# MDProject/Binary-Fluctuating-Lattice-Boltzmann

Hardware: AMD Instinct MI355X
Metric: MLUPS (million lattice-site updates/sec) D3Q19×2 at 256³/512³; % HBM roofline (higher is better)
Workload: dtype f64; 1 GPU; 512x512x512 periodic, stripe init, zero noise; schedule=handover, slab_per_gpu=512x512x512, parallelism=single GPU

## Files before the change

binary-fluctuating-lattice-boltzmann_amd/_lib.py:

```python
import ctypes
import os

_HERE = os.path.dirname(os.path.abspath(__file__))
LIB_PATH = os.environ.get("BFLBM_LIB", os.path.join(_HERE, "csrc", "libbflbm.so"))

NVEL = 19
NHYDRO = 22
NHYDROBAR = 9
TRACE_NREC = 12
HALO_STATE, HALO_NEXT, HALO_UPLOAD = 0, 1, 2


class Params(ctypes.Structure):
    _fields_ = [
        ("tau_f", ctypes.c_double), ("tau_g", ctypes.c_double),
        ("alpha0", ctypes.c_double), ("alpha1", ctypes.c_double),
        ("kappa", ctypes.c_double), ("kBT", ctypes.c_double), ("cs2", ctypes.c_double),
        ("rho_lo", ctypes.c_double), ("rho_hi", ctypes.c_double),
        ("seed", ctypes.c_uint64),
    ]


class Domain(ctypes.Structure):
    _fields_ = [
# ... 40 lines not shown
    "bflbm_ring_set_overlap": (ctypes.c_int, [_vp, ctypes.c_int]),
    "bflbm_ring_set_transport": (ctypes.c_int, [_vp, ctypes.c_int]),
    "bflbm_ring_last_transport": (ctypes.c_int, [_vp, _P(ctypes.c_int), _P(ctypes.c_int)]),
    "bflbm_debug_addresses": (ctypes.c_int, [_vp, _P(ctypes.c_ulonglong)]),
    "bflbm_tune_placement": (ctypes.c_int, [_vp, ctypes.c_int, _P(ctypes.c_float), _P(ctypes.c_int)]),
    "bflbm_placement_report": (ctypes.c_int, [_vp, _P(ctypes.c_float), _P(ctypes.c_int), _P(ctypes.c_int)]),
    "bflbm_state_total_max": (ctypes.c_int, [_vp, _dp]),
    "bflbm_set_state_total_max": (ctypes.c_int, [_vp, ctypes.c_double]),
    "bflbm_step_boundary": (ctypes.c_int, [_vp]),
    "bflbm_step_interior": (ctypes.c_int, [_vp]),
    "bflbm_step_finish": (ctypes.c_int, [_vp]),
    "bflbm_halo_bytes": (ctypes.c_int, [_vp, ctypes.c_int, _P(ctypes.c_size_t)]),
    "bflbm_halo_pack": (ctypes.c_int, [_vp, ctypes.c_int, ctypes.c_int, _vp]),
    "bflbm_halo_unpack": (ctypes.c_int, [_vp, ctypes.c_int, ctypes.c_int, _vp]),
    "bflbm_halo_planes": (ctypes.c_int, [_vp, ctypes.c_int, ctypes.c_int, ctypes.c_int, _P(_vp), _P(ctypes.c_size_t), _P(ctypes.c_int)]),
    "bflbm_ring_create": (ctypes.c_int, [_P(Params), _P(ctypes.c_int), ctypes.c_int, _P(ctypes.c_int), ctypes.c_int, _P(_vp)]),
    "bflbm_ring_destroy": (ctypes.c_int, [_vp]),
    "bflbm_ring_size": (ctypes.c_int, [_vp, _P(ctypes.c_int)]),
    "bflbm_ring_slab": (ctypes.c_int, [_vp, ctypes.c_int, _P(_vp)]),
    "bflbm_ring_set_params": (ctypes.c_int, [_vp, _P(Params)]),
    "bflbm_ring_set_schedule": (ctypes.c_int, [_vp, ctypes.c_int]),
    "bflbm_ring_init_mixture": (ctypes.c_int, [_vp]),
    "bflbm_ring_init_stripe": (ctypes.c_int, [_vp, ctypes.c_double]),
    "bflbm_ring_init_droplet": (ctypes.c_int, [_vp, ctypes.c_double]),
    "bflbm_ring_commit_upload": (ctypes.c_int, [_vp, ctypes.c_int]),
    "bflbm_ring_step": (ctypes.c_int, [_vp, ctypes.c_int]),
    "bflbm_ring_com_sums": (ctypes.c_int, [_vp, _dp]),
    "bflbm_ring_mass": (ctypes.c_int, [_vp, _dp, _dp]),
    "bflbm_ring_sync": (ctypes.c_int, [_vp]),
    "bflbm_ring_set_ref_state": (ctypes.c_int, [_vp, _vp, _vp, _vp, _P(Fab)]),
    "bflbm_ring_enable_ref_state": (ctypes.c_int, [_vp, ctypes.c_int, _dp]),
    "bflbm_ring_prepare_ref": (ctypes.c_int, [_vp]),
    "bflbm_batch_create": (ctypes.c_int, [_P(Params), ctypes.c_int, _P(ctypes.c_int), ctypes.c_int, _P(_vp)]),
    "bflbm_batch_destroy": (ctypes.c_int, [_vp]),
    "bflbm_batch_size": (ctypes.c_int, [_vp, _P(ctypes.c_int)]),
    "bflbm_batch_replica": (ctypes.c_int, [_vp, ctypes.c_int, _P(_vp)]),
    "bflbm_batch_set_schedule": (ctypes.c_int, [_vp, ctypes.c_int]),
    "bflbm_batch_resolved_schedule": (ctypes.c_int, [_vp, _P(ctypes.c_int)]),
    "bflbm_batch_step": (ctypes.c_int, [_vp, ctypes.c_int]),
    "bflbm_batch_sync": (ctypes.c_int, [_vp]),
    "bflbm_trace_create": (ctypes.c_int, [_vp, ctypes.c_int, ctypes.c_longlong, ctypes.c_double, _P(_vp)]),
    "bflbm_batch_trace_create": (ctypes.c_int, [_vp, ctypes.c_int, ctypes.c_longlong, ctypes.c_double, _P(_vp)]),
    "bflbm_trace_destroy": (ctypes.c_int, [_vp]),
    "bflbm_trace_sample": (ctypes.c_int, [_vp]),
    "bflbm_trace_reset": (ctypes.c_int, [_vp]),
    "bflbm_trace_count": (ctypes.c_int, [_vp, _P(ctypes.c_longlong), _P(ctypes.c_int)]),
    "bflbm_trace_read": (ctypes.c_int, [_vp, ctypes.c_longlong, ctypes.c_longlong, _vp, _vp]),
    "bflbm_set_ref_state": (ctypes.c_int, [_vp, _vp, _vp, _vp, _P(Fab)]),
    "bflbm_enable_ref_state": (ctypes.c_int, [_vp, ctypes.c_int, _dp]),
    "bflbm_ref_state_active": (ctypes.c_int, [_vp, _P(ctypes.c_int)]),
    "bflbm_set_com": (ctypes.c_int, [_vp, _dp]),
    "bflbm_get_hydrovsbar": (ctypes.c_int, [_vp, _vp, ctypes.c_int, _P(Fab)]),
    "bflbm_get_hydrovs": (ctypes.c_int, [_vp, _vp, ctypes.c_int, _P(Fab)]),
    "bflbm_get_noise": (ctypes.c_int, [_vp, _vp, _vp, _P(Fab)]),
    "bflbm_inject_noise": (ctypes.c_int, [_vp, _vp, _vp, _P(Fab)]),
    "bflbm_com_sums": (ctypes.c_int, [_vp, _dp]),
    "bflbm_mass": (ctypes.c_int, [_vp, _dp, _dp]),
    "bflbm_sync": (ctypes.c_int, [_vp]),
    "bflbm_droplet_moments": (ctypes.c_int, [_vp, _dp]),
    "bflbm_ring_droplet_moments": (ctypes.c_int, [_vp, _dp]),
    "bflbm_fit_droplet": (ctypes.c_int, [_vp, _dp, _dp, ctypes.c_int, ctypes.c_double, _dp, _P(ctypes.c_int)]),
    "bflbm_ring_fit_droplet": (ctypes.c_int, [_vp, _dp, _dp, ctypes.c_int, ctypes.c_double, _dp, _P(ctypes.c_int)]),
    "bflbm_flowfit_default_opts": (None, [_P(FlowFitOpts)]),
    "bflbm_fit_droplet_flow": (ctypes.c_int, [_vp, _P(FlowFitOpts), _dp, _P(ctypes.c_int)]),
    "bflbm_ring_fit_droplet_flow": (ctypes.c_int, [_vp, _P(FlowFitOpts), _dp, _P(ctypes.c_int)]),
    "bflbm_flowfit_coefficients": (ctypes.c_int, [ctypes.c_double] * 6 + [_dp]),
    "bflbm_sf_create": (ctypes.c_int, [_vp, ctypes.c_int, _P(ctypes.c_int), _P(ctypes.c_int), _dp, _P(_vp)]),
    "bflbm_sf_destroy": (ctypes.c_int, [_vp]),
    "bflbm_sf_reset": (ctypes.c_int, [_vp]),
    "bflbm_sf_accumulate": (ctypes.c_int, [_vp, ctypes.c_int, ctypes.c_int]),
    "bflbm_sf_nsamples": (ctypes.c_int, [_vp, _P(ctypes.c_longlong)]),
    "bflbm_sf_get": (ctypes.c_int, [_vp, ctypes.c_int, ctypes.c_int, _vp]),
    "bflbm_ring_sf_create": (ctypes.c_int, [_vp, ctypes.c_int, _P(ctypes.c_int), _P(ctypes.c_int), _dp, _P(_vp)]),
    "bflbm_ring_sf_destroy": (ctypes.c_int, [_vp]),
    "bflbm_ring_sf_reset": (ctypes.c_int, [_vp]),
    "bflbm_ring_sf_accumulate": (ctypes.c_int, [_vp, ctypes.c_int, ctypes.c_int]),
    "bflbm_ring_sf_nsamples": (ctypes.c_int, [_vp, _P(ctypes.c_longlong)]),
    "bflbm_ring_sf_get": (ctypes.c_int, [_vp, ctypes.c_int, ctypes.c_int, _vp]),
    "bflbm_timer_start": (ctypes.c_int, [_vp]),
    "bflbm_timer_stop": (ctypes.c_int, [_vp, _P(ctypes.c_float)]),
    "bflbm_rng_site_normals": (ctypes.c_int, [ctypes.c_uint64, ctypes.c_uint64, ctypes.c_uint32, _dp]),
    "bflbm_debug_time_kernel": (ctypes.c_int, [_vp, ctypes.c_int, ctypes.c_int, _P(ctypes.c_float)]),
    "bflbm_device_bytes": (ctypes.c_int, [_vp, _P(ctypes.c_size_t)]),
}


class BflbmError(RuntimeError):
    pass


_lib = None


def load():
    global _lib
    if _lib is not None:
        return _lib
    if not os.path.exists(LIB_PATH):
        raise BflbmError(
            f"{LIB_PATH} not found: build the HIP extension first "
            "(python -c 'import __graft_entry__ as g; g.build()' or make -C "
            f"{os.path.dirname(LIB_PATH)}). There is no CPU fallback.")
    if os.environ.get("BFLBM_NO_TORCH") != "1":
        try:
            import torch
        except ImportError:
            pass
    lib = ctypes.CDLL(LIB_PATH)
    for name, (res, args) in SIGNATURES.items():
        fn = getattr(lib, name)
        fn.restype = res
        fn.argtypes = args
    if lib.bflbm_abi_version() != 1:
        raise BflbmError("libbflbm.so ABI version mismatch")
    _lib = lib
    return lib


def check(rc):
    if rc != 0:
        msg = load().bflbm_last_error()
        raise BflbmError(msg.decode() if msg else f"bflbm call failed ({rc})")
```

binary-fluctuating-lattice-boltzmann_amd/csrc/bflbm.hip:

```cpp
#include <hip/hip_runtime.h>
#include <algorithm>
#include <array>
#include <cmath>
#include <cstdarg>
#include <cstdio>
#include <cstring>
#include <limits>
#include <string>
#include <thread>
#include <vector>

#include "../../include/bflbm.h"
#define BFLBM_NHYDRO_ 22
#include "bflbm_kernels.h"
#include "bflbm_fused.h"
#include "bflbm_handover.h"
#include "bflbm_batch.h"

namespace {

thread_local std::string g_err;

int fail(const char* fmt, ...) {
  char buf[512];
// ... 955 lines not shown
  return 0;
}

int bflbm_ref_state_active(const bflbm_ctx* c, int* active) {
  if (!c || !active) return fail("null argument");
  *active = ref_active(c) ? 1 : 0;
  return 0;
}

int bflbm_set_com(bflbm_ctx* c, const double com[3]) {
  if (!c || !com) return fail("null argument");
  BFLBM_REFUSE_OPEN_STEP(c, "bflbm_set_com");
  for (int d = 0; d < 3; ++d) if (!std::isfinite(com[d])) return fail("bflbm_set_com: centre of mass is not finite");
  for (int d = 0; d < 3; ++d) c->com[d] = com[d];
  c->com_valid = true;
  return 0;
}

int bflbm_sync(bflbm_ctx* c) {
  if (!c) return fail("null context");
  HIP_TRY(hipSetDevice(c->dom.device));
  HIP_TRY(hipStreamSynchronize(c->stream));
  return 0;
}

int bflbm_timer_start(bflbm_ctx* c) {
  if (!c) return fail("null context");
  HIP_TRY(hipEventRecord(c->ev0, c->stream));
  return 0;
}
int bflbm_timer_stop(bflbm_ctx* c, float* ms) {
  if (!c || !ms) return fail("null argument");
  HIP_TRY(hipEventRecord(c->ev1, c->stream));
  HIP_TRY(hipEventSynchronize(c->ev1));
  HIP_TRY(hipEventElapsedTime(ms, c->ev0, c->ev1));
  return 0;
}

int bflbm_rng_site_normals(uint64_t seed, uint64_t site, uint32_t noise_index, double* out36) {
  if (!out36) return fail("null argument");
  static const double tab[BFLBM_NORMAL_TABLE_N] = BFLBM_NORMAL_TABLE_VALUES;
  bflbm_rng_state st;
  bflbm_rng_seed((uint32_t)seed, (uint32_t)(seed >> 32), site, noise_index, st);
  for (int k = 0; k < 36; ++k) out36[k] = (k < 33) ? bflbm_normal_from_bits(bflbm_rng_next(st), tab) : 0.;
  return 0;
}

int bflbm_debug_time_kernel(bflbm_ctx* c, int which, int reps, float* ms) {
  if (!c || !ms || reps < 1) return fail("bad argument");
  if (c->step_open()) return fail("diagnostics inside an open step");
  HIP_TRY(hipSetDevice(c->dom.device));
  const size_t sbytes = (size_t)2 * Q * c->G.vol * sizeof(double);
  for (int r = -1; r < reps; ++r) {
    if (r == 0) HIP_TRY(hipEventRecord(c->ev0, c->stream));
    if (which == 0) hipLaunchKernelGGL(k_pull, plane_grid(c, c->nzl), dim3(256), 0, c->stream, c->S[c->cur], c->S[1 - c->cur], c->G, own_lo(c));
    else if (which == 1) hipLaunchKernelGGL(k_density, plane_grid(c, c->nzl), dim3(256), 0, c->stream, c->S[c->cur], c->rho, c->phi, c->G, own_lo(c));
    else if (which == 2) HIP_TRY(hipMemcpyAsync(c->S[1 - c->cur], c->S[c->cur], sbytes, hipMemcpyDeviceToDevice, c->stream));
    else return fail("unknown diagnostic kernel %d", which);
  }
  HIP_TRY(hipGetLastError());
  HIP_TRY(hipEventRecord(c->ev1, c->stream));
  HIP_TRY(hipEventSynchronize(c->ev1));
  float t = 0.f;
  HIP_TRY(hipEventElapsedTime(&t, c->ev0, c->ev1));
  *ms = t / reps;
  halos_written(c);
  return 0;
}


int bflbm_debug_addresses(const bflbm_ctx* c, unsigned long long out[8]) {
  if (!c || !out) return fail("null argument");
  out[0] = (unsigned long long)c->S[0]; out[1] = (unsigned long long)c->S[1]; out[2] = (unsigned long long)c->rho; out[3] = (unsigned long long)c->phi;
  out[4] = (unsigned long long)c->partial; out[5] = (unsigned long long)c->frames[0]; out[6] = (unsigned long long)c->frames[1]; out[7] = (unsigned long long)c->G.vol;
  return 0;
}

int bflbm_device_bytes(const bflbm_ctx* c, size_t* bytes) {
  if (!c || !bytes) return fail("null argument");
  *bytes = c->bytes;
  return 0;
}


struct bflbm_ring {
  std::vector<bflbm_ctx*> ctx;
  std::vector<hipStream_t> comm;
  std::vector<hipEvent_t> packed;
  std::vector<hipEvent_t> unpacked;
  std::vector<std::array<bool, 2>> peer_ok;
  size_t bytes = 0;
  bool overlap = true;
  int transport = 0;
  int last_kernel_faces = 0, last_copy_faces = 0;
};

static int ring_mark(bflbm_ring* r) {
  const int n = (int)r->ctx.size();
  if (n == 1) return 0;
  for (int k = 0; k < n; ++k) {
    bflbm_ctx* c = r->ctx[k];
    HIP_TRY(hipSetDevice(c->dom.device));
    HIP_TRY(hipEventRecord(r->packed[k], c->stream));
  }
  return 0;
}
static int ring_copy(bflbm_ring* r, int kind) {
  const int n = (int)r->ctx.size();
  if (n == 1) return 0;
  r->last_kernel_faces = r->last_copy_faces = 0;
  for (int k = 0; k < n; ++k) {
    bflbm_ctx* c = r->ctx[k];
    const int lower = (k + n - 1) % n, upper = (k + 1) % n;
    HIP_TRY(hipSetDevice(c->dom.device));
    HIP_TRY(hipStreamWaitEvent(r->comm[k], r->packed[lower], 0));
    HIP_TRY(hipStreamWaitEvent(r->comm[k], r->packed[upper], 0));
    HIP_TRY(hipStreamWaitEvent(r->comm[k], r->packed[k], 0));
    const size_t pbytes = (size_t)c->G.plane * sizeof(double);
    for (int side = 0; side < 2; ++side) {
      bflbm_ctx* src = r->ctx[side == 0 ? lower : upper];
      HaloTable Tu, Tp;
      halo_table(c, kind, side, false, Tu);
      halo_table(src, kind, 1 - side, true, Tp);
      double* dst_base = halo_buffer(c, kind);
      const double* src_base = halo_buffer(src, kind);
      for (int e = 0; e < 2 * Q; ++e) if (Tu.comp[e] != Tp.comp[e]) return fail("halo tables of neighbouring slabs disagree");
      static const bool force_copies = [] { const char* e = getenv("BFLBM_RING_COPY_FALLBACK"); return e && atoi(e) != 0; }();
      const bool reachable = !force_copies && r->transport == 0 && ((src->dom.device == c->dom.device) || r->peer_ok[k][side]);
      if (reachable && (c->G.plane % 2 == 0) && (c->G.vol % 2 == 0) && (src->G.vol % 2 == 0)) {
        ++r->last_kernel_faces;
        dim3 g((unsigned)((c->G.plane / 2 + 255) / 256), (unsigned)(2 * Q));
        hipLaunchKernelGGL(k_halo_pull, g, dim3(256), 0, r->comm[k], dst_base, src_base, c->G.plane, c->G.vol, src->G.vol, Tu, Tp);
        HIP_TRY(hipGetLastError());
      } else {
        ++r->last_copy_faces;
        for (int e = 0; e < 2 * Q; ++e) {
          double* d = dst_base + (size_t)Tu.comp[e] * c->G.vol + (size_t)Tu.plane[e] * c->G.plane;
          const double* sp = src_base + (size_t)Tp.comp[e] * src->G.vol + (size_t)Tp.plane[e] * src->G.plane;
          HIP_TRY(hipMemcpyPeerAsync(d, c->dom.device, sp, src->dom.device, pbytes, r->comm[k]));
        }
      }
    }
    HIP_TRY(hipEventRecord(r->unpacked[k], r->comm[k]));
    if (kind == BFLBM_HALO_STATE) halos_written(c);
  }
  return 0;
}
static int ring_exchange(bflbm_ring* r, int kind) { return ring_mark(r) || ring_copy(r, kind); }

static int ring_join(bflbm_ring* r) {
  const int n = (int)r->ctx.size();
  if (n == 1) return 0;
  for (int k = 0; k < n; ++k) {
    HIP_TRY(hipSetDevice(r->ctx[k]->dom.device));
    HIP_TRY(hipStreamWaitEvent(r->ctx[k]->stream, r->unpacked[k], 0));
    HIP_TRY(hipStreamWaitEvent(r->ctx[k]->stream, r->unpacked[(k + 1) % n], 0));
    HIP_TRY(hipStreamWaitEvent(r->ctx[k]->stream, r->unpacked[(k + n - 1) % n], 0));
  }
  return 0;
}

int bflbm_ring_create(const bflbm_params* p, const int n[3], int nslabs, const int* devices, int ndevices, bflbm_ring** out) {
  if (!p || !n || !out || nslabs < 1) return fail("bflbm_ring_create: bad argument");
  if (nslabs > 1 && n[2] / nslabs < 4) return fail("bflbm_ring_create: every slab needs at least 4 planes");
  bflbm_ring* r = new bflbm_ring();
  for (int k = 0; k < nslabs; ++k) {
// ... 365 lines not shown
```

binary-fluctuating-lattice-boltzmann_amd/csrc/bflbm_handover_body.inc:

```
  using L = HoLayout<TY>;
  constexpr int TX = 64, NT = TX * TY;
  constexpr int LW = TX + 2, LSZ = (TX + 2) * (TY + 2);
  constexpr int NRING = 2 * (TX + 2) + 2 * TY;
  static_assert(TY >= 4 && 4 + 2 * TY <= 64 && 8 * TY <= 64, "tile shape");
  __shared__ double rp[4][2][LSZ];
  __shared__ double gl[Q][NT];
  __shared__ double fl[Q][NT];
  __shared__ double exch[2][2][2][2][TX];
  __shared__ double accs[2][2][2][TX];
  __shared__ double colacc[2][2][2][TY][6];
  __shared__ double colfin[2][2][2][TY][6];

  __shared__ double ntab[MODE == 1 ? BFLBM_NORMAL_TABLE_N : 4];

  int col, chunk;
  if (!fused_map(F, (int)blockIdx.x, col, chunk)) return;
  if (MODE == 1) d_load_normal_table(ntab, true);
  const int tix = col % F.ntx;
  int tiy = col / F.ntx + F.row0;
  if (tiy >= F.nty) tiy -= F.nty;
  const int x0 = tix * TX, y0 = tiy * TY;
  const int tid = threadIdx.x;
  const int lane = tid & 63;
  const int ty = __builtin_amdgcn_readfirstlane(tid >> 6);
// ... 48 lines not shown
    }
  }

  const int qa = F.pa + chunk * F.cstride;
  const int qb = min(F.pb, qa + F.lz);
  auto wrapp = [&](int q) {
    if (!G.zwrap) return q;
    const int m = q % G.nzs;
    return m < 0 ? m + G.nzs : m;
  };
  const int fa = qa + 1, fb = qb - 2;

  double anb[2][2] = {{0., 0.}, {0., 0.}};
  double aup[2][2] = {{0., 0.}, {0., 0.}};

  auto finish = [&](int tpf, int rb) {
    if (tpf < fa || tpf > fb) return;
    double* __restrict__ fp = Hg.fout + (long long)tpf * Hg.fplane;
    if (!RAG) {
      if (edge_row) {
#pragma unroll
        for (int k = 0; k < 2; ++k) {
          const double e = exch[rb][k][side_y][0][lane] + exch[rb][k][side_y][1][lane];
          st(fp, tile_rec + (unsigned)(k * L::FR + (side_y ? L::ET : L::EB) + lane) * 8u, e);
        }
      }
    } else {
#pragma unroll
      for (int k = 0; k < 2; ++k) {
        if (r_bot) st(fp, tile_rec + (unsigned)(k * L::FR + L::EB + lane) * 8u, exch[rb][k][0][0][lane] + exch[rb][k][0][1][lane]);
        if (r_top) st(fp, tile_rec + (unsigned)(k * L::FR + L::ET + lane) * 8u, exch[rb][k][1][0][lane] + exch[rb][k][1][1][lane]);
      }
    }
    if (ty == 0 && lane < 8 * TY) {
      const int k = lane / (4 * TY), rem = lane % (4 * TY), sd = rem / (2 * TY), u = rem % (2 * TY);
      const int ne = ah > 2 ? ah - 2 : 0;
      double v = 0.; int slot = -1;
      if (u < ne) {
        const int row = u + 1;
        v = colfin[rb][k][sd][row][0] + colfin[rb][k][sd][row - 1][1] + colfin[rb][k][sd][row + 1][2];
        slot = (sd ? L::ER : L::EL) + row - 1;
      } else if (u - ne < ah + 2) {
        const int row = u - ne - 1;
        if (row >= 0 && row < ah) v = colfin[rb][k][sd][row][3];
        if (row - 1 >= 0 && row - 1 < ah) v += colfin[rb][k][sd][row - 1][4];
        if (row + 1 >= 0 && row + 1 < ah) v += colfin[rb][k][sd][row + 1][5];
        slot = (sd ? L::OR_ : L::OL) + row + 1;
      }
      if (slot >= 0) st(fp, tile_rec + (unsigned)(k * L::FR + slot) * 8u, v);
    }
  };

  auto pull_plane = [&](int q, double (&f)[Q], double (&g)[Q], double (&hv)[2][4], const int which = 0, const int parts = 3) {
    const double* __restrict__ pl[3] = { S + (long long)wrapp(q - 1) * G.plane, S + (long long)wrapp(q) * G.plane,
                                         S + (long long)wrapp(q + 1) * G.plane };
    unsigned oo[3][3];
#pragma unroll
    for (int a = 0; a < 3; ++a)
#pragma unroll
      for (int b2 = 0; b2 < 3; ++b2) { oo[a][b2] = yo[a] + xo[b2]; asm volatile("" : "+v"(oo[a][b2])); }
    if (parts & 1) {
#pragma unroll
      for (int i = 0; i < Q; ++i) {
        const double* __restrict__ b = pl[1 - Vel::cz[i]] + (long long)i * G.vol;
        const unsigned o = oo[1 - Vel::cy[i]][1 - Vel::cx[i]];
        if (which != 2) f[i] = ld(b, o);
        if (which != 1) g[i] = ld(b + (long long)Q * G.vol, o);
      }
    }
    if ((parts & 2) && which != 2 && Hg.use_frames && q >= fa && q <= fb && has_rtask) {
      const double* __restrict__ fp = Hg.fin + (long long)q * Hg.fplane;
#pragma unroll
      for (int j = 0; j < 4; ++j) {
        unsigned o = fo[j];
        asm volatile("" : "+v"(o));
        if (j < 2 || j < nfo) { hv[0][j] = ld(fp, o); hv[1][j] = ld(fp + L::FR, o); }
        else { hv[0][j] = 0.; hv[1][j] = 0.; }
      }
    }
  };
  double nf[Q], ng[Q], hvn[2][4];
  constexpr bool DEFER_G = UNIT && MODE == 0 && !RAG;
  double dg[Q];
  pull_plane(qa - 1, nf, ng, hvn);
  __builtin_amdgcn_s_waitcnt(0x0F70);

  int it = 0;
  auto position = [&](const int q, auto col_c, auto ldn_c, auto pend_c, auto keep_c) {
    constexpr bool do_collide = decltype(col_c)::value, load_next = decltype(ldn_c)::value;
    constexpr bool pending = decltype(pend_c)::value, keep = decltype(keep_c)::value;
    constexpr bool spread_f = do_collide && load_next;
    const int slot = it & 3;
    const double* __restrict__ pl[3] = { S + (long long)wrapp(q - 1) * G.plane, S + (long long)wrapp(q) * G.plane,
                                         S + (long long)wrapp(q + 1) * G.plane };
    double cf[Q], cg[Q], hv[2][4];
#pragma unroll
    for (int i = 0; i < Q; ++i) { cf[i] = nf[i]; cg[i] = ng[i]; }
#pragma unroll
    for (int j = 0; j < 4; ++j) { hv[0][j] = hvn[0][j]; hv[1][j] = hvn[1][j]; }
    const bool ring_from_frames = Hg.use_frames && q >= fa && q <= fb;
    double zero = 0.0;
    asm volatile("" : "+v"(zero));
    auto density = [&](const double (&fs)[Q]) { double r = zero;
#pragma unroll
      for (int i = 0; i < Q; ++i) r += fs[i];
      return r; };
    if (ring_from_frames) {
      if (active) { rp[slot][0][lown] = density(cf); rp[slot][1][lown] = density(cg); }
      if (has_rtask) {
        double r0 = hv[0][0] + hv[0][1], r1 = hv[1][0] + hv[1][1];
        if (nfo > 2) { r0 += hv[0][2]; r1 += hv[1][2]; }
        if (nfo > 3) { r0 += hv[0][3]; r1 += hv[1][3]; }
        rp[slot][0][lhalo] = r0; rp[slot][1][lhalo] = r1;
      }
    } else {
      if (active) { rp[slot][0][lown] = density(cf); rp[slot][1][lown] = density(cg); }
      if (tid < (RAG ? 2 * (aw + 2) + 2 * ah : NRING)) {
        const int r = tid;
        int rx, ry;
        if (r < aw + 2) { rx = r; ry = 0; }
        else if (r < 2 * (aw + 2)) { rx = r - (aw + 2); ry = ah + 1; }
        else if (r < 2 * (aw + 2) + ah) { rx = 0; ry = r - 2 * (aw + 2) + 1; }
        else { rx = aw + 1; ry = r - 2 * (aw + 2) - ah + 1; }
        const int hx = wrapx(x0 + rx - 1), hy = wrapy(y0 + ry - 1);
        const unsigned hxo[3] = { (unsigned)wrapx(hx - 1) * 8u, (unsigned)hx * 8u, (unsigned)wrapx(hx + 1) * 8u };
        const unsigned hyo[3] = { (unsigned)(wrapy(hy - 1) * G.pitch) * 8u, (unsigned)(hy * G.pitch) * 8u, (unsigned)(wrapy(hy + 1) * G.pitch) * 8u };
        double t[2][Q];
#pragma unroll
        for (int i = 0; i < Q; ++i) {
          unsigned o = hyo[1 - Vel::cy[i]] + hxo[1 - Vel::cx[i]];
          asm volatile("" : "+v"(o));
          const double* __restrict__ b = pl[1 - Vel::cz[i]] + (long long)i * G.vol;
          t[0][i] = ld(b, o);
          t[1][i] = ld(b + (long long)Q * G.vol, o);
        }
        __builtin_amdgcn_sched_barrier(0);
        rp[slot][0][ry * LW + rx] = density(t[0]);
        rp[slot][1][ry * LW + rx] = density(t[1]);
      }
    }
    if (pending) {
      double* __restrict__ Dq = D + (long long)wrapp(q - 2) * G.plane + (long long)Q * G.vol;
      unsigned oq = yo[1] + xo[1];
#pragma unroll
      for (int i = 0; i < Q; ++i) {
        if (!ho_g_deferred(i)) continue;
        asm volatile("" : "+v"(oq));
        __builtin_nontemporal_store(dg[i], reinterpret_cast<double*>(reinterpret_cast<char*>(Dq + (long long)i * G.vol) + oq));
      }
    }
    __syncthreads();
    finish(q - 3, (it & 1) ^ 1);
    const int pc = q - 1;
    double mg[Q], jg[3];
    if (do_collide) {
      double pg[Q];
#pragma unroll
      for (int i = 0; i < Q; ++i) pg[i] = gl[i][tid];
      d_moments(pg, mg);
      d_momentum(pg, jg);
    }
    double mf[Q], jf[3];
    if (do_collide) {
      double pfl[Q];
#pragma unroll
      for (int i = 0; i < Q; ++i) pfl[i] = fl[i][tid];
      d_moments(pfl, mf);
      d_momentum(pfl, jf);
    }
#pragma unroll
    for (int i = 0; i < Q; ++i) gl[i][tid] = cg[i];
#pragma unroll
    for (int i = 0; i < Q; ++i) fl[i][tid] = cf[i];
    if (load_next) pull_plane(q + 1, nf, ng, hvn, 1, spread_f ? 2 : 3);
    if (do_collide) {
      const int sl[3] = { (it - 2) & 3, (it - 1) & 3, it & 3 };
      const double r = rp[sl[1]][0][lown], ph = rp[sl[1]][1][lown];
      double nb[Q], grad_rho[3], grad_phi[3];
#pragma unroll
      for (int i = 0; i < Q; ++i) nb[i] = rp[sl[1 + Vel::cz[i]]][0][lown + Vel::cy[i] * LW + Vel::cx[i]];
      d_gradient(P, nb, grad_rho);
#pragma unroll
      for (int i = 0; i < Q; ++i) nb[i] = rp[sl[1 + Vel::cz[i]]][1][lown + Vel::cy[i] * LW + Vel::cx[i]];
      d_gradient(P, nb, grad_phi);
      const int pcw = wrapp(pc);
      double fn3[3] = {0., 0., 0.}, gn3[3] = {0., 0., 0.};
      NoiseAmp NA; bflbm_rng_state rst;
      if (MODE == 1) {
        d_noise_amp(P, r, ph, r + ph, NA);
        d_noise_head(P, NA, global_site(G, x, y, pcw), noise_index, ntab, rst, fn3);
#pragma unroll
        for (int k3 = 0; k3 < 3; ++k3) gn3[k3] = -fn3[k3];
      }
      double* __restrict__ Dp = D + (long long)pcw * G.plane;
      unsigned o = yo[1] + xo[1];
      asm volatile("" : "+v"(o));
      SiteHydro Hy;
      SiteRecip R;
      d_site_recips(P, r, ph, R);
      d_hydrovars_j(P, jf, jg, r, ph, grad_rho, grad_phi, fn3, gn3, Hy, R);
      double v_b[3];
      d_barycentric(r, ph, Hy, v_b, R);
      const int tp = pc - 1;
      const bool tp_ok = tp >= fa && tp <= fb;
      double* __restrict__ fp = Hg.fout + (long long)tp * Hg.fplane;
      const int wb = it & 1;
      const double zn[Q] = {0.};
      auto finish_fluid = [&](const double (&mom)[Q], const int k, auto later_c) {
        PopTerms T;
        d_population_terms(mom, T);
        double* __restrict__ Dk = Dp + (long long)(k * Q) * G.vol;
        auto put = [&](int i, double v) {
          if (decltype(later_c)::value && ho_g_deferred(i)) { dg[i] = v; return; }
          if (active) __builtin_nontemporal_store(v, reinterpret_cast<double*>(reinterpret_cast<char*>(Dk + (long long)i * G.vol) + o));
        };
        auto shr = [&](double v) { return ho_shr((RAG && !active_x) ? 0.0 : v); };
        auto shl = [&](double v) { return ho_shl((RAG && !active_x) ? 0.0 : v); };
        auto diag = [&](int g, int j) {
          return j == 0 ? T.B[g] + T.p[g] + T.q[g] + T.r[g] : j == 1 ? T.B[g] - T.p[g] - T.q[g] + T.r[g]
               : j == 2 ? T.B[g] + T.p[g] - T.q[g] - T.r[g] : T.B[g] - T.p[g] + T.q[g] - T.r[g]; };
        const double o0 = T.rest, o1 = T.E[0] + T.O[0], o2 = T.E[0] - T.O[0];
        put(0, o0); put(1, o1); put(2, o2);
        const double x00 = o0 + shr(o1) + shl(o2);
        const double o3 = T.E[1] + T.O[1], o7 = diag(0, 0), o10 = diag(0, 3);
        put(3, o3); put(7, o7); put(10, o10);
        const double xp0 = o3 + shr(o7) + shl(o10);
        const double o4 = T.E[1] - T.O[1], o9 = diag(0, 2), o8 = diag(0, 1);
        put(4, o4); put(9, o9); put(8, o8);
        const double xm0 = o4 + shr(o9) + shl(o8);
        const double o5 = T.E[2] + T.O[2], o15 = diag(2, 0), o18 = diag(2, 2);
        put(5, o5); put(15, o15); put(18, o18);
        const double x0p = o5 + shr(o15) + shl(o18);
        const double o6 = T.E[2] - T.O[2], o17 = diag(2, 3), o16 = diag(2, 1);
        put(6, o6); put(17, o17); put(16, o16);
        const double x0m = o6 + shr(o17) + shl(o16);
        const double o11 = diag(1, 0), o12 = diag(1, 1), o13 = diag(1, 2), o14 = diag(1, 3);
        put(11, o11); put(12, o12); put(13, o13); put(14, o14);
        const double oxp = side_x ? o15 : o18, ox0 = side_x ? o1 : o2, oxm = side_x ? o17 : o16, oyp = side_x ? o7 : o10, oym = side_x ? o9 : o8;
        if (!RAG) {
        const double np = row_down ? o14 : o11, n0 = row_down ? xm0 : xp0, nm = row_down ? o12 : o13;
        const double fin_nb = anb[k][1] + nm;
        anb[k][1] = anb[k][0] + n0;
        anb[k][0] = np;
        double hand = fin_nb;
        if (is_edge) {
          const double fin_self = accs[1][k][side_y][lane] + x0m;
          accs[1][k][side_y][lane] = accs[0][k][side_y][lane] + x00;
          accs[0][k][side_y][lane] = x0p;
          hand = fin_self;
          if (tp_ok) st(fp, tile_rec + (unsigned)(k * L::FR + (side_y ? L::OT : L::OB) + lane) * 8u, fin_nb);
        }
        if (TY == 4 || row_kind) exch[wb][k][side_y][edge_row ? 0 : 1][lane] = hand;
        } else {
        const double fin_dn = anb[k][1] + o12;
        anb[k][1] = anb[k][0] + xm0;
        anb[k][0] = o14;
        const double fin_up = aup[k][1] + o13;
        aup[k][1] = aup[k][0] + xp0;
        aup[k][0] = o11;
        if (r_bot || r_top) {
          const int sd = r_bot ? 0 : 1;
          const double fin_self = accs[1][k][sd][lane] + x0m;
          accs[1][k][sd][lane] = accs[0][k][sd][lane] + x00;
          accs[0][k][sd][lane] = x0p;
          if (r_bot) { exch[wb][k][0][0][lane] = fin_self; if (tp_ok) st(fp, tile_rec + (unsigned)(k * L::FR + L::OB + lane) * 8u, fin_dn); }
          if (r_top) { exch[wb][k][1][0][lane] = fin_self; if (tp_ok) st(fp, tile_rec + (unsigned)(k * L::FR + L::OT + lane) * 8u, fin_up); }
        }
        if (r_hdn) exch[wb][k][0][1][lane] = fin_dn;
        if (r_hup) exch[wb][k][1][1][lane] = fin_up;
        }
        if (col_lane) {
          const double vp[6] = { x0p, o11, o14, oxp, 0., 0. };
          const double v0[6] = { x00, xp0, xm0, ox0, oyp, oym };
          const double vm[6] = { x0m, o13, o12, oxm, 0., 0. };
#pragma unroll
          for (int j = 0; j < 6; ++j) {
            colfin[wb][k][side_x][ty][j] = colacc[1][k][side_x][ty][j] + vm[j];
            colacc[1][k][side_x][ty][j] = colacc[0][k][side_x][ty][j] + v0[j];
            colacc[0][k][side_x][ty][j] = vp[j];
          }
        }
      };
      if (spread_f) pull_plane(q + 1, nf, ng, hvn, 1, 1);
      if (MODE == 1) d_relax_generated(P, mf, r, v_b, Hy.uf, Hy.af, P.inv_tau_f_bar, fn3, NA.sr, ntab, rst, R.cs4);
      else           d_relax<false, UNIT>(P, mf, r, v_b, Hy.uf, Hy.af, P.inv_tau_f_bar, zn, R.cs4);
      if (spread_f) {
#pragma unroll
        for (int s_ = 0; s_ < Q; ++s_) {
          __builtin_amdgcn_sched_group_barrier(0x020, 1, 0);
          __builtin_amdgcn_sched_group_barrier(0x002, MODE == 1 ? HO_SPREAD_F1 : (UNIT ? (RAG ? HO_SPREAD_FU_RAG : HO_SPREAD_FU) : HO_SPREAD_F), 0);
        }
      }
      finish_fluid(mf, 0, std::false_type{});
      if (load_next) pull_plane(q + 1, nf, ng, hvn, 2);
      if (MODE == 1) d_relax_generated(P, mg, ph, v_b, Hy.ug, Hy.ag, P.inv_tau_g_bar, gn3, NA.sp, ntab, rst, R.cs4);
      else           d_relax<false, UNIT>(P, mg, ph, v_b, Hy.ug, Hy.ag, P.inv_tau_g_bar, zn, R.cs4);
      finish_fluid(mg, 1, std::bool_constant<keep>{});
    } else if (load_next) {
      pull_plane(q + 1, nf, ng, hvn, 2);
      __builtin_amdgcn_s_waitcnt(0x0F70);
    }
  };
  using T_ = std::true_type; using F_ = std::false_type;
  {
    int q = qa - 1;
    for (int k = 0; k < 2; ++k, ++q, ++it) position(q, F_{}, T_{}, F_{}, F_{});
    if constexpr (DEFER_G) {
      if (q < qb) {
        position(q, T_{}, T_{}, F_{}, T_{});
        ++q; ++it;
        for (; q < qb; ++q, ++it) position(q, T_{}, T_{}, T_{}, T_{});
        position(qb, T_{}, F_{}, T_{}, F_{});
      } else {
        position(qb, T_{}, F_{}, F_{}, F_{});
      }
    } else {
      for (; q < qb; ++q, ++it) position(q, T_{}, T_{}, F_{}, F_{});
      position(qb, T_{}, F_{}, F_{}, F_{});
    }
    ++it;
  }
  __syncthreads();
  finish(qb - 2, (it & 1) ^ 1);
```

binary-fluctuating-lattice-boltzmann_amd/lattice.py:

```python
import ctypes

import numpy as np

from . import _lib
from ._lib import Domain, Fab, Params, NVEL, NHYDRO, NHYDROBAR, check


def default_params(**overrides):
    p = Params()
    _lib.load().bflbm_default_params(ctypes.byref(p))
    for k, v in overrides.items():
        if not hasattr(p, k):
            raise AttributeError(f"unknown model parameter {k!r}")
        setattr(p, k, v)
    return p


def make_fab(lo, hi, vlo=None, vhi=None):
    f = Fab()
    vlo = lo if vlo is None else vlo
    vhi = hi if vhi is None else vhi
    for d in range(3):
        f.lo[d], f.hi[d], f.vlo[d], f.vhi[d] = int(lo[d]), int(hi[d]), int(vlo[d]), int(vhi[d])
    return f
# ... 302 lines not shown
        s = (ctypes.c_double * 4)()
        check(self.lib.bflbm_com_sums(self._h, s))
        return np.array(list(s))

    def update_com(self):
        s = self.com_sums()
        return s[1:] / s[0]

    def mass(self):
        r, p = ctypes.c_double(), ctypes.c_double()
        check(self.lib.bflbm_mass(self._h, ctypes.byref(r), ctypes.byref(p)))
        return r.value, p.value

    def set_ref_state(self, rho_eq, phi_eq, rhot_eq, com_ref, fab=None):
        n = self.n
        fab = fab if fab is not None else make_fab((0, 0, 0), (n[0] - 1, n[1] - 1, n[2] - 1))
        arrs = [np.ascontiguousarray(a, dtype=np.float64) for a in (rho_eq, phi_eq, rhot_eq)]
        check(self.lib.bflbm_set_ref_state(self._h, _ptr(arrs[0]), _ptr(arrs[1]), _ptr(arrs[2]), ctypes.byref(fab)))
        c = (ctypes.c_double * 3)(*[float(v) for v in com_ref])
        check(self.lib.bflbm_enable_ref_state(self._h, 1, c))

    def disable_ref_state(self):
        check(self.lib.bflbm_enable_ref_state(self._h, 0, None))

    @property
    def ref_state_active(self):
        a = ctypes.c_int()
        check(self.lib.bflbm_ref_state_active(self._h, ctypes.byref(a)))
        return bool(a.value)

    def set_com(self, com):
        c = (ctypes.c_double * 3)(*[float(v) for v in com])
        check(self.lib.bflbm_set_com(self._h, c))

    def halo_bytes(self, kind=_lib.HALO_STATE):
        n = ctypes.c_size_t()
        check(self.lib.bflbm_halo_bytes(self._h, int(kind), ctypes.byref(n)))
        return n.value

    def halo_pack(self, kind, side, device_ptr):
        check(self.lib.bflbm_halo_pack(self._h, int(kind), int(side), ctypes.c_void_p(device_ptr)))

    def halo_unpack(self, kind, side, device_ptr):
        check(self.lib.bflbm_halo_unpack(self._h, int(kind), int(side), ctypes.c_void_p(device_ptr)))

    def halo_planes(self, kind, side, pack):
        ptrs = (ctypes.c_void_p * 64)()
        nb, cnt = ctypes.c_size_t(), ctypes.c_int()
        check(self.lib.bflbm_halo_planes(self._h, int(kind), int(side), int(bool(pack)), ptrs, ctypes.byref(nb), ctypes.byref(cnt)))
        return [int(ptrs[k]) for k in range(cnt.value)], nb.value

    def halo_plane_tensors(self, kind, side, pack, device):
        import torch
        cache = self.__dict__.setdefault("_plane_views", {})
        ptrs, nb = self.halo_planes(kind, side, pack)
        out = []
        for p in ptrs:
            t = cache.get(p)
            if t is None:
                t = cache[p] = torch.as_tensor(_DevicePlane(p, nb // 8), device=device)
            out.append(t)
        return out

    def sync(self):
        check(self.lib.bflbm_sync(self._h))

    def timer_start(self):
        check(self.lib.bflbm_timer_start(self._h))

    def timer_stop(self):
        ms = ctypes.c_float()
        check(self.lib.bflbm_timer_stop(self._h, ctypes.byref(ms)))
        return ms.value

    def debug_time_kernel(self, which, reps=10):
        ms = ctypes.c_float()
        check(self.lib.bflbm_debug_time_kernel(self._h, int(which), int(reps), ctypes.byref(ms)))
        return ms.value

    def device_bytes(self):
        n = ctypes.c_size_t()
        check(self.lib.bflbm_device_bytes(self._h, ctypes.byref(n)))
        return n.value


class RingLBM(_DropletMixin):
    _droplet_fn = ("bflbm_ring_droplet_moments", "bflbm_ring_fit_droplet", "bflbm_ring_fit_droplet_flow")

    """The whole lattice as a ring of z-slabs driven by this one process through the native ring of the
    C-ABI (bflbm_ring_*): slab r on GPU devices[r % len(devices)], halo exchange by peer copies overlapped
    with the interior planes.  Same operator surface as BinaryLBM; fields are full-lattice arrays."""

    def __init__(self, nx, ny=None, nz=None, nslabs=1, devices=(0,), params=None, schedule=None):
        self.lib = _lib.load()
        ny = nx if ny is None else ny
        nz = nx if nz is None else nz
        self.n = (int(nx), int(ny), int(nz))
        self.params = params if params is not None else default_params()
        n3 = (ctypes.c_int * 3)(*self.n)
        dev = (ctypes.c_int * len(devices))(*[int(d) for d in devices])
        h = ctypes.c_void_p()
        check(self.lib.bflbm_ring_create(ctypes.byref(self.params), n3, int(nslabs), dev, len(devices), ctypes.byref(h)))
        self._h = h
        self.slabs = []
        for r in range(int(nslabs)):
            c = ctypes.c_void_p()
            check(self.lib.bflbm_ring_slab(self._h, r, ctypes.byref(c)))
            z0, z1 = (self.n[2] * r) // nslabs, (self.n[2] * (r + 1)) // nslabs
            self.slabs.append(BinaryLBM._borrow(c, self.n, z0, z1, r, nslabs, self.params))
        if schedule is not None:
            code = SCHEDULES.get(schedule, schedule)
            check(self.lib.bflbm_ring_set_schedule(self._h, int(code)))

    def close(self):
        if getattr(self, "_h", None):
            for d in list(getattr(self, "_dependents", [])):
                d.close()
            for s in self.slabs:
                for d in list(getattr(s, "_dependents", [])):
                    d.close()
            self.lib.bflbm_ring_destroy(self._h)
            self._h = None
            for s in self.slabs:
                s._h = None

    def __del__(self):
        try:
            self.close()
        except Exception:
            pass

    def set_params(self, **kw):
        for k, v in kw.items():
            if not hasattr(self.params, k):
                raise AttributeError(f"unknown model parameter {k!r}")
            setattr(self.params, k, v)
        check(self.lib.bflbm_ring_set_params(self._h, ctypes.byref(self.params)))

    def LBM_init_mixture(self):
        check(self.lib.bflbm_ring_init_mixture(self._h))

    def LBM_init_stripe(self, frac):
        check(self.lib.bflbm_ring_init_stripe(self._h, float(frac)))

    def LBM_init_droplet(self, r):
        check(self.lib.bflbm_ring_init_droplet(self._h, float(r)))

    def LBM_init(self, f0, g0):
        _check_array(f0, NVEL, (self.n[2], self.n[1], self.n[0]), "f0")
        _check_array(g0, NVEL, (self.n[2], self.n[1], self.n[0]), "g0")
        fab = make_fab((0, 0, 0), (self.n[0] - 1, self.n[1] - 1, self.n[2] - 1))
        for s in self.slabs:
            s.upload(f0, g0, fab)
        check(self.lib.bflbm_ring_commit_upload(self._h, 1))

    def LBM_timestep(self, nsteps=1):
        check(self.lib.bflbm_ring_step(self._h, int(nsteps)))

    def _gather(self, ncomp, call):
        out = np.empty((ncomp, self.n[2], self.n[1], self.n[0]))
        fab = make_fab((0, 0, 0), (self.n[0] - 1, self.n[1] - 1, self.n[2] - 1))
        for s in self.slabs:
            call(s, out, fab)
        return out

    def populations(self):
# ... 171 lines not shown
```

include/bflbm.h:

```cpp
#ifndef BFLBM_H_
#define BFLBM_H_

#include <stddef.h>
#include <stdint.h>

#ifdef __cplusplus
extern "C" {
#endif

#define BFLBM_NVEL 19
#define BFLBM_NHYDRO 22
#define BFLBM_NHYDROBAR 9
#define BFLBM_ABI_VERSION 1

typedef struct bflbm_params {
  double tau_f, tau_g;
  double alpha0, alpha1;
  double kappa;
  double kBT;
  double cs2;
  double rho_lo, rho_hi;
  uint64_t seed;
} bflbm_params;

// ... 82 lines not shown
int bflbm_ring_enable_ref_state(bflbm_ring* r, int on, const double com_ref[3]);
int bflbm_ring_prepare_ref(bflbm_ring* r);

typedef struct bflbm_batch bflbm_batch;
int bflbm_batch_create(const bflbm_params* p , int nreplicas, const int n[3], int device, bflbm_batch** out);
int bflbm_batch_destroy(bflbm_batch* b);
int bflbm_batch_size(const bflbm_batch* b, int* nreplicas);
int bflbm_batch_replica(bflbm_batch* b, int r, bflbm_ctx** ctx);
int bflbm_batch_set_schedule(bflbm_batch* b, int schedule);
int bflbm_batch_resolved_schedule(const bflbm_batch* b, int* schedule);
int bflbm_batch_step(bflbm_batch* b, int nsteps);
int bflbm_batch_sync(bflbm_batch* b);

typedef struct bflbm_trace bflbm_trace;
#define BFLBM_TRACE_NREC 12
int bflbm_trace_create(bflbm_ctx* c, int every, long long capacity, double threshold, bflbm_trace** out);
int bflbm_batch_trace_create(bflbm_batch* b, int every, long long capacity, double threshold, bflbm_trace** out);
int bflbm_trace_destroy(bflbm_trace* t);
int bflbm_trace_sample(bflbm_trace* t);
int bflbm_trace_reset(bflbm_trace* t);
int bflbm_trace_count(const bflbm_trace* t, long long* nsamples, int* nreplicas);
int bflbm_trace_read(bflbm_trace* t, long long first, long long count,
                     double* rec   ,
                     long long* steps );

int bflbm_get_hydrovsbar(bflbm_ctx* c, double* dst, int ncomp, const bflbm_fab* box);
int bflbm_get_hydrovs(bflbm_ctx* c, double* dst, int ncomp, const bflbm_fab* box);
int bflbm_get_noise(bflbm_ctx* c, double* fnoise, double* gnoise, const bflbm_fab* box);

int bflbm_inject_noise(bflbm_ctx* c, const double* fnoise, const double* gnoise, const bflbm_fab* box);

int bflbm_com_sums(bflbm_ctx* c, double sums[4]);

int bflbm_mass(bflbm_ctx* c, double* rho_sum, double* phi_sum);

int bflbm_set_ref_state(bflbm_ctx* c, const double* rho_eq, const double* phi_eq, const double* rhot_eq, const bflbm_fab* box);
int bflbm_enable_ref_state(bflbm_ctx* c, int on, const double com_ref[3]);
int bflbm_ref_state_active(const bflbm_ctx* c, int* active);
int bflbm_set_com(bflbm_ctx* c, const double com[3]);

int bflbm_sync(bflbm_ctx* c);

typedef struct bflbm_sf bflbm_sf;
int bflbm_sf_create(bflbm_ctx* c, int npairs, const int* var_a, const int* var_b, const double* scale, bflbm_sf** out);
int bflbm_sf_destroy(bflbm_sf* s);
int bflbm_sf_reset(bflbm_sf* s);
int bflbm_sf_accumulate(bflbm_sf* s, int lb_hydrovars, int reset);
int bflbm_sf_nsamples(const bflbm_sf* s, long long* n);
int bflbm_sf_get(bflbm_sf* s, int what, int zero_avg, double* dst);

typedef struct bflbm_ring_sf bflbm_ring_sf;
int bflbm_ring_sf_create(bflbm_ring* r, int npairs, const int* var_a, const int* var_b, const double* scale, bflbm_ring_sf** out);
int bflbm_ring_sf_destroy(bflbm_ring_sf* s);
int bflbm_ring_sf_reset(bflbm_ring_sf* s);
int bflbm_ring_sf_accumulate(bflbm_ring_sf* s, int lb_hydrovars, int reset);
int bflbm_ring_sf_nsamples(const bflbm_ring_sf* s, long long* n);
int bflbm_ring_sf_get(bflbm_ring_sf* s, int what, int zero_avg, double* dst);

int bflbm_droplet_moments(bflbm_ctx* c, double moments[20]);
int bflbm_ring_droplet_moments(bflbm_ring* r, double moments[20]);
int bflbm_fit_droplet(bflbm_ctx* c, const double r0[3], double params[4], int max_iter, double tol, double* cost, int* iterations);
int bflbm_ring_fit_droplet(bflbm_ring* r, const double r0[3], double params[4], int max_iter, double tol, double* cost, int* iterations);

typedef struct {
  double W0, R0, eta_W, eta_R, dt, undul_ratio;
  int nstep, step_window, max_retry;
} bflbm_flowfit_opts;
void bflbm_flowfit_default_opts(bflbm_flowfit_opts* o);
int bflbm_fit_droplet_flow(bflbm_ctx* c, const bflbm_flowfit_opts* opts, double result[3], int* retries);
int bflbm_ring_fit_droplet_flow(bflbm_ring* r, const bflbm_flowfit_opts* opts, double result[3], int* retries);
int bflbm_flowfit_coefficients(double W, double R, double eta_W, double eta_R, double dt, double C0, double out[9]);

int bflbm_timer_start(bflbm_ctx* c);
int bflbm_timer_stop(bflbm_ctx* c, float* ms);

int bflbm_rng_site_normals(uint64_t seed, uint64_t site, uint32_t noise_index, double* out36);

int bflbm_debug_time_kernel(bflbm_ctx* c, int which, int reps, float* ms_per_launch);

int bflbm_tune_placement(bflbm_ctx* c, int max_candidates, float* ms_per_step, int* kept);
int bflbm_placement_report(const bflbm_ctx* c, float ms_per_step[8], int* tried, int* kept);
int bflbm_debug_addresses(const bflbm_ctx* c, unsigned long long out[8]);
int bflbm_device_bytes(const bflbm_ctx* c, size_t* bytes);

#ifdef __cplusplus
}
#endif
#endif
```

Baseline: 8923 MLUPS.

## Restructure handover chunk prologue/epilogue to prefetch halo ring densities ahead

Replaces the per-chunk prologue with an explicit warm-up that loads two planes and their halo-ring densities together, so the ring loads overlap with the interior pulls. The last planes of each chunk get specialised tail variants that issue ring loads for the next plane during the current plane's relaxation, instead of computing the ring at the start of each plane. It also adds a query API that reports the chunk plan. The aim is to hide halo-ring gather latency at chunk edges. The cost is extra register pressure from the nr buffers and more template instantiations of the position lambda.

```diff
diff --git a/binary-fluctuating-lattice-boltzmann_amd/_lib.py b/binary-fluctuating-lattice-boltzmann_amd/_lib.py
--- a/binary-fluctuating-lattice-boltzmann_amd/_lib.py
+++ b/binary-fluctuating-lattice-boltzmann_amd/_lib.py
@@ -146,6 +146,7 @@
     "bflbm_rng_site_normals": (ctypes.c_int, [ctypes.c_uint64, ctypes.c_uint64, ctypes.c_uint32, _dp]),
     "bflbm_debug_time_kernel": (ctypes.c_int, [_vp, ctypes.c_int, ctypes.c_int, _P(ctypes.c_float)]),
     "bflbm_device_bytes": (ctypes.c_int, [_vp, _P(ctypes.c_size_t)]),
+    "bflbm_handover_chunks": (ctypes.c_int, [_vp, _P(ctypes.c_int)]),
 }
 
 
diff --git a/binary-fluctuating-lattice-boltzmann_amd/csrc/bflbm.hip b/binary-fluctuating-lattice-boltzmann_amd/csrc/bflbm.hip
--- a/binary-fluctuating-lattice-boltzmann_amd/csrc/bflbm.hip
+++ b/binary-fluctuating-lattice-boltzmann_amd/csrc/bflbm.hip
@@ -1061,6 +1061,16 @@
   return 0;
 }
 
+int bflbm_handover_chunks(const bflbm_ctx* c, int plan[3]) {
+  if (!c || !plan) return fail("null argument");
+  const HoSig& s = c->fsig[c->cur][0];
+  plan[0] = plan[1] = plan[2] = 0;
+  if (s.lz <= 0) return 0;
+  plan[0] = s.lz; plan[1] = s.nchunks;
+  plan[2] = std::min(s.pb, s.pa + (s.nchunks - 1) * s.cstride + s.lz) - (s.pa + (s.nchunks - 1) * s.cstride);
+  return 0;
+}
+
 
 struct bflbm_ring {
   std::vector<bflbm_ctx*> ctx;
diff --git a/binary-fluctuating-lattice-boltzmann_amd/csrc/bflbm_handover_body.inc b/binary-fluctuating-lattice-boltzmann_amd/csrc/bflbm_handover_body.inc
--- a/binary-fluctuating-lattice-boltzmann_amd/csrc/bflbm_handover_body.inc
+++ b/binary-fluctuating-lattice-boltzmann_amd/csrc/bflbm_handover_body.inc
@@ -154,13 +154,54 @@
   double nf[Q], ng[Q], hvn[2][4];
   constexpr bool DEFER_G = UNIT && MODE == 0 && !RAG;
   double dg[Q];
-  pull_plane(qa - 1, nf, ng, hvn);
-  __builtin_amdgcn_s_waitcnt(0x0F70);
+  const int nring = RAG ? 2 * (aw + 2) + 2 * ah : NRING;
+  int prx, pry;
+  if (tid < aw + 2) { prx = tid; pry = 0; }
+  else if (tid < 2 * (aw + 2)) { prx = tid - (aw + 2); pry = ah + 1; }
+  else if (tid < 2 * (aw + 2) + ah) { prx = 0; pry = tid - 2 * (aw + 2) + 1; }
+  else { prx = aw + 1; pry = tid - 2 * (aw + 2) - ah + 1; }
+  const int pring = pry * LW + prx;
+  auto ring_request = [&](int q, double (&t)[2][Q]) {
+    if (tid < nring) {
+      const double* __restrict__ pl[3] = { S + (long long)wrapp(q - 1) * G.plane, S + (long long)wrapp(q) * G.plane,
+                                           S + (long long)wrapp(q + 1) * G.plane };
+      const int hx = wrapx(x0 + prx - 1), hy = wrapy(y0 + pry - 1);
+      const unsigned hxo[3] = { (unsigned)wrapx(hx - 1) * 8u, (unsigned)hx * 8u, (unsigned)wrapx(hx + 1) * 8u };
+      const unsigned hyo[3] = { (unsigned)(wrapy(hy - 1) * G.pitch) * 8u, (unsigned)(hy * G.pitch) * 8u, (unsigned)(wrapy(hy + 1) * G.pitch) * 8u };
+#pragma unroll
+      for (int i = 0; i < Q; ++i) {
+        unsigned o = hyo[1 - Vel::cy[i]] + hxo[1 - Vel::cx[i]];
+        asm volatile("" : "+v"(o));
+        const double* __restrict__ b = pl[1 - Vel::cz[i]] + (long long)i * G.vol;
+        t[0][i] = ld(b, o);
+        t[1][i] = ld(b + (long long)Q * G.vol, o);
+      }
+    } else {
+#pragma unroll
+      for (int i = 0; i < Q; ++i) { t[0][i] = 0.; t[1][i] = 0.; }
+    }
+  };
+  auto ring_store = [&](int slot, const double (&t)[2][Q]) {
+    if (tid < nring) {
+      double zero = 0.0;
+      asm volatile("" : "+v"(zero));
+#pragma unroll
+      for (int k = 0; k < 2; ++k) {
+        double r = zero;
+#pragma unroll
+        for (int i = 0; i < Q; ++i) r += t[k][i];
+        rp[slot][k][pring] = r;
+      }
+    }
+  };
+  double nr[2][Q];
 
   int it = 0;
-  auto position = [&](const int q, auto col_c, auto ldn_c, auto pend_c, auto keep_c) {
+  auto position = [&](const int q, auto col_c, auto ldn_c, auto pend_c, auto keep_c, auto tail_c, const bool pend_rt) {
     constexpr bool do_collide = decltype(col_c)::value, load_next = decltype(ldn_c)::value;
     constexpr bool pending = decltype(pend_c)::value, keep = decltype(keep_c)::value;
+    constexpr int tail = decltype(tail_c)::value;
+    constexpr bool ring_pre = tail >= 2, ring_nxt = tail == 1 || tail == 2;
     constexpr bool spread_f = do_collide && load_next;
     const int slot = it & 3;
     const double* __restrict__ pl[3] = { S + (long long)wrapp(q - 1) * G.plane, S + (long long)wrapp(q) * G.plane,
@@ -177,7 +218,10 @@
 #pragma unroll
       for (int i = 0; i < Q; ++i) r += fs[i];
       return r; };
-    if (ring_from_frames) {
+    if (ring_pre) {
+      if (active) { rp[slot][0][lown] = density(cf); rp[slot][1][lown] = density(cg); }
+      ring_store(slot, nr);
+    } else if (ring_from_frames) {
       if (active) { rp[slot][0][lown] = density(cf); rp[slot][1][lown] = density(cg); }
       if (has_rtask) {
         double r0 = hv[0][0] + hv[0][1], r1 = hv[1][0] + hv[1][1];
@@ -211,7 +255,7 @@
         rp[slot][1][ry * LW + rx] = density(t[1]);
       }
     }
-    if (pending) {
+    if (pending || (DEFER_G && tail != 0 && pend_rt)) {
       double* __restrict__ Dq = D + (long long)wrapp(q - 2) * G.plane + (long long)Q * G.vol;
       unsigned oq = yo[1] + xo[1];
 #pragma unroll
@@ -365,6 +409,11 @@
       }
       finish_fluid(mf, 0, std::false_type{});
       if (load_next) pull_plane(q + 1, nf, ng, hvn, 2);
+      if (ring_nxt) {
+        __builtin_amdgcn_sched_barrier(0);
+        ring_request(q + 1, nr);
+        __builtin_amdgcn_sched_barrier(0);
+      }
       if (MODE == 1) d_relax_generated(P, mg, ph, v_b, Hy.ug, Hy.ag, P.inv_tau_g_bar, gn3, NA.sp, ntab, rst, R.cs4);
       else           d_relax<false, UNIT>(P, mg, ph, v_b, Hy.ug, Hy.ag, P.inv_tau_g_bar, zn, R.cs4);
       finish_fluid(mg, 1, std::bool_constant<keep>{});
@@ -374,22 +423,58 @@
     }
   };
   using T_ = std::true_type; using F_ = std::false_type;
+  using N0 = std::integral_constant<int, 0>; using N1 = std::integral_constant<int, 1>;
+  using N2 = std::integral_constant<int, 2>; using N3 = std::integral_constant<int, 3>;
   {
-    int q = qa - 1;
-    for (int k = 0; k < 2; ++k, ++q, ++it) position(q, F_{}, T_{}, F_{}, F_{});
-    if constexpr (DEFER_G) {
-      if (q < qb) {
-        position(q, T_{}, T_{}, F_{}, T_{});
-        ++q; ++it;
-        for (; q < qb; ++q, ++it) position(q, T_{}, T_{}, T_{}, T_{});
-        position(qb, T_{}, F_{}, T_{}, F_{});
+    const bool short_chunk = qb - qa <= 2;
+    {
+      double af[Q], ag[Q], ta[2][Q];
+      pull_plane(qa - 1, af, ag, hvn, 0, 1);
+      ring_request(qa - 1, ta);
+      pull_plane(qa, nf, ng, hvn, 0, 1);
+      __builtin_amdgcn_s_waitcnt(0x0F70);
+      double zero = 0.0;
+      asm volatile("" : "+v"(zero));
+      auto density = [&](const double (&fs)[Q]) { double r = zero;
+#pragma unroll
+        for (int i = 0; i < Q; ++i) r += fs[i];
+        return r; };
+      if (active) { rp[0][0][lown] = density(af); rp[0][1][lown] = density(ag); }
+      ring_store(0, ta);
+      if (active) { rp[1][0][lown] = density(nf); rp[1][1][lown] = density(ng); }
+#pragma unroll
+      for (int i = 0; i < Q; ++i) gl[i][tid] = ng[i];
+#pragma unroll
+      for (int i = 0; i < Q; ++i) fl[i][tid] = nf[i];
+      __builtin_amdgcn_sched_barrier(0);
+      ring_request(qa, ta);
+      pull_plane(qa + 1, nf, ng, hvn);
+      if (short_chunk) ring_request(qa + 1, nr);
+      __builtin_amdgcn_s_waitcnt(0x0F70);
+      ring_store(1, ta);
+    }
+    int q = qa + 1;
+    it = 2;
+    asm volatile("" : "+s"(it), "+s"(q));
+    bool have_dg = false;
+    int qe = qb - 2;
+    asm volatile("" : "+s"(qe));
+    if (!short_chunk) {
+      if constexpr (DEFER_G) {
+        if (q < qe) {
+          position(q, T_{}, T_{}, F_{}, T_{}, N0{}, false);
+          ++q; ++it;
+          for (; q < qe; ++q, ++it) position(q, T_{}, T_{}, T_{}, T_{}, N0{}, false);
+          have_dg = true;
+        }
       } else {
-        position(qb, T_{}, F_{}, F_{}, F_{});
-      }
-    } else {
-      for (; q < qb; ++q, ++it) position(q, T_{}, T_{}, F_{}, F_{});
-      position(qb, T_{}, F_{}, F_{}, F_{});
-    }
+        for (; q < qe; ++q, ++it) position(q, T_{}, T_{}, F_{}, F_{}, N0{}, false);
+      }
+      position(q, T_{}, T_{}, F_{}, std::bool_constant<DEFER_G>{}, N1{}, have_dg);
+      have_dg = DEFER_G; ++q; ++it;
+    }
+    if (q == qb - 1) { position(q, T_{}, T_{}, F_{}, std::bool_constant<DEFER_G>{}, N2{}, have_dg); have_dg = DEFER_G; ++q; ++it; }
+    position(qb, T_{}, F_{}, F_{}, F_{}, N3{}, have_dg);
     ++it;
   }
   __syncthreads();
diff --git a/binary-fluctuating-lattice-boltzmann_amd/lattice.py b/binary-fluctuating-lattice-boltzmann_amd/lattice.py
--- a/binary-fluctuating-lattice-boltzmann_amd/lattice.py
+++ b/binary-fluctuating-lattice-boltzmann_amd/lattice.py
@@ -408,6 +408,11 @@
         n = ctypes.c_size_t()
         check(self.lib.bflbm_device_bytes(self._h, ctypes.byref(n)))
         return n.value
+
+    def handover_chunks(self):
+        plan = (ctypes.c_int * 3)()
+        check(self.lib.bflbm_handover_chunks(self._h, plan))
+        return tuple(plan)
 
 
 class RingLBM(_DropletMixin):
diff --git a/include/bflbm.h b/include/bflbm.h
--- a/include/bflbm.h
+++ b/include/bflbm.h
@@ -188,6 +188,7 @@
 int bflbm_placement_report(const bflbm_ctx* c, float ms_per_step[8], int* tried, int* kept);
 int bflbm_debug_addresses(const bflbm_ctx* c, unsigned long long out[8]);
 int bflbm_device_bytes(const bflbm_ctx* c, size_t* bytes);
+int bflbm_handover_chunks(const bflbm_ctx* c, int plan[3]);
 
 #ifdef __cplusplus
 }
```

After: 8947 MLUPS, median of 6. Within noise of the previous version (+0.3%).
